# victorca25/traiNNer

Hardware: AMD Instinct MI355X
Metric: HR images/sec (G+D step), ESRGAN x4 128->512 (higher is better)
Workload: dtype f32 (bf16x3)

## Files before the change

### include/trainner_hip.h

```cpp
#ifndef TRAINNER_HIP_H
#define TRAINNER_HIP_H

#include <stdint.h>

#ifdef __cplusplus
extern "C" {
#endif

#define TNR_OK 0
#define TNR_EINVAL (-1)
#define TNR_ELAUNCH (-2)

enum { TNR_ACT_NONE = 0, TNR_ACT_LRELU = 1, TNR_ACT_RELU = 2 };

enum {
    TNR_CONV_3x3 = 0,
    TNR_CONV_3x3_UP2 = 1,
    TNR_CONV_4x4_S2 = 2,
    TNR_DGRAD_4x4_S2 = 3,
    TNR_CONV_1x1 = 4,
    TNR_CONV_3x3_C4 = 5,
    TNR_CONV_7x7_C4 = 6
};

enum {
    TNR_PACK_FWD = 0,
    TNR_PACK_DGRAD_3x3 = 1,
    TNR_PACK_FWD_S2D = 2,
    TNR_PACK_DGRAD_S2 = 3,
    TNR_PACK_COL_FWD = 4,
    TNR_PACK_COL_DGRAD3 = 5,
    TNR_PACK_C4_FWD = 6,
    TNR_PACK_C4_DGRAD3 = 7
};

#define TNR_MMA_F32 0
#define TNR_MMA_BF16 1
#define TNR_MMA_BF16X3 2

typedef struct tnr_view {
    float *ptr;
    int32_t ctot;
    int32_t coff;
} tnr_view;

typedef struct tnr_conv_desc {
    tnr_view x;
    int32_t N, H, W;
    int32_t Cin;
    const float *wp;
    int32_t KinP, KoutP;
    tnr_view y;
    int32_t Ho, Wo, Cout;
    int32_t mode;
    const float *bias;
    int32_t act;
// ... 74 lines not shown
int tnr_conv_sweep_pack_batch(const tnr_sweep_pack_item *items_dev, int32_t n, int32_t max_units, void *stream);
int tnr_conv_sweep(const tnr_conv_desc *stages, int32_t n, const void *image, uint32_t *ws, int64_t ws_bytes, uint32_t epoch,
                   void *stream);
int64_t tnr_conv_thin_pack_floats(int32_t reduce_channels);
int tnr_conv_thin_pack(const float *w_oihw, float *wp, int32_t Cout, int32_t Cin, int32_t dgrad, void *stream);
int tnr_conv_thin(tnr_view x, int32_t N, int32_t H, int32_t W, int32_t Cin, const float *wp, tnr_view y, int32_t Cout,
                  const float *bias, float alpha, void *stream);
int64_t tnr_conv_thin7_pack_floats(int32_t reduce_channels);
int tnr_conv_thin7_pack(const float *w_oihw, float *wp, int32_t Cout, int32_t Cin, int32_t dgrad, void *stream);
int tnr_conv_thin7(tnr_view x, int32_t N, int32_t H, int32_t W, int32_t Cin, const float *wp, tnr_view y, int32_t Ho, int32_t Wo,
                   int32_t Cout, int32_t pad, int32_t reflect, const float *bias, float alpha, void *stream);
int64_t tnr_wgrad_workspace_bytes(const tnr_wgrad_desc *d);
int64_t tnr_wgrad_thin_workspace_bytes(int32_t N, int32_t H, int32_t Cbig);
int tnr_wgrad_thin(tnr_view big, tnr_view small, int32_t N, int32_t H, int32_t W, int32_t Cbig, int32_t Csmall, int32_t flip,
                   float *dw, float *db, float alpha, float beta, float *ws, int64_t ws_bytes, void *stream);
int64_t tnr_wgrad_thin7_workspace_bytes(int32_t N, int32_t Hbig_grid, int32_t Cbig);
int tnr_wgrad_thin7(tnr_view big, int32_t N, int32_t H, int32_t W, int32_t rpad, tnr_view small, int32_t Hs, int32_t Ws, int32_t off,
                    int32_t Cbig, int32_t Csmall, int32_t flip, float *dw, float *db, float alpha, float beta, float *ws, int64_t ws_bytes,
                    void *stream);
int tnr_conv_wgrad(const tnr_wgrad_desc *d, void *stream);
#define TNR_WGRAD_GROUP_MAX 12
int tnr_conv_wgrad_group(const tnr_wgrad_desc *descs, int32_t n, void *stream);
int tnr_wgrad_tile_class(const tnr_wgrad_desc *d, int32_t group_jobs, int32_t x3_occ, int32_t out[12]);

int tnr_gconv_fwd(tnr_view x, int32_t N, int32_t H, int32_t W, int32_t Cin, const float *w, const float *bias, tnr_view y, int32_t Ho,
                  int32_t Wo, int32_t Cout, int32_t k, int32_t stride, int32_t pad, int32_t reflect, int32_t act, float slope, void *stream);
int tnr_gconv_dgrad(tnr_view g, int32_t N, int32_t H, int32_t W, int32_t Cin, const float *w, tnr_view gx, int32_t Ho, int32_t Wo,
                    int32_t Cout, int32_t k, int32_t stride, int32_t pad, int32_t reflect, void *stream);
int64_t tnr_gconv_wgrad_workspace_bytes(int32_t Cout, int32_t Cin, int32_t k);
int tnr_gconv_wgrad(tnr_view x, int32_t N, int32_t H, int32_t W, int32_t Cin, tnr_view g, int32_t Ho, int32_t Wo, int32_t Cout, int32_t k,
                    int32_t stride, int32_t pad, int32_t reflect, float *dw, float *db, float alpha, float beta, double *ws,
                    int64_t ws_bytes, void *stream);
int tnr_bias_grad(tnr_view g, int64_t pixels, int32_t C, float *db, float alpha, float beta, double *ws, int64_t ws_bytes, void *stream);
int tnr_pad2d(tnr_view x, tnr_view y, int32_t N, int32_t H, int32_t W, int32_t C, int32_t pad, int32_t mode, void *stream);
int tnr_unpad2d(tnr_view xp, tnr_view y, int32_t N, int32_t H, int32_t W, int32_t C, int32_t pad, int32_t mode, void *stream);
int tnr_window2d(tnr_view src, int32_t Hs, int32_t Ws, tnr_view dst, int32_t N, int32_t Hd, int32_t Wd, int32_t C, int32_t oy,
                 int32_t ox, int32_t acc, void *stream);
int tnr_tanh_fwd(const float *x, float *y, int64_t n, void *stream);
int tnr_tanh_bwd(const float *g, const float *y, float *gx, int64_t n, void *stream);
int tnr_gan_loss(const float *pred, int64_t n, int32_t type, float target, float *out, float *grad, void *stream);
int tnr_dp_unique_id(void *id128);
int tnr_dp_init(const void *id128, int32_t rank, int32_t world, void **comm);
int tnr_dp_allreduce_bucket(void *comm, float *buf, int64_t count, int32_t average, void *stream);
int tnr_dp_broadcast(void *comm, float *buf, int64_t count, int32_t root, void *stream);
int tnr_dp_comm_count(void *comm, int32_t *nranks);
int tnr_dp_finalize(void *comm);
// ... 178 lines not shown
```

### trainner_amd/csrc/conv_sweep.hip

```cpp
#include <stddef.h>
#include <string.h>
#include <type_traits>
#include <utility>
#include "conv_body.h"
#include "conv_epilogue.h"
#include "conv_handoff.h"

namespace {

constexpr int SW_TH = 8, SW_TW = 32, SW_HT = SW_TH + 2, SW_WT = SW_TW + 2;
constexpr int SW_ROW = TNR_X3_ROW;
constexpr int SW_A_ROWS = SW_HT * SW_WT;
constexpr int SW_A_ALLOC_ROWS = 384;
constexpr int SW_A_FLOATS = SW_A_ALLOC_ROWS * SW_ROW;
constexpr int SW_UNIT_FLOATS = 32 * SW_ROW;
constexpr int SW_SLOT_UNITS = 9;
constexpr int SW_SLOT_FLOATS = SW_SLOT_UNITS * SW_UNIT_FLOATS;
constexpr int SW_RING = 3;
constexpr size_t SW_LDS_BYTES = (size_t)(2 * SW_A_FLOATS + SW_RING * SW_SLOT_FLOATS) * sizeof(float);
constexpr int SW_NPASS = 9, SW_NSTAGE = 5, SW_NTILE = 6;
constexpr int SW_A_IT = (SW_A_ROWS * 4 + 511) / 512;
constexpr int SW_B_PIECES = (SW_SLOT_UNITS * 3 + 7) / 8;
static_assert(SW_LDS_BYTES <= 160 * 1024, "one sweep workgroup per CU");

// ... 1455 lines not shown
    const int form = sweep_form();
    if (n == SW4_NSTAGE) {
        TNR_REQUIRE(form == 5, "conv_sweep: four stages run in the direct four-wave form only");
        hipLaunchKernelGGL((conv_sweep4_kernel<true, false, SwPlan4>), dim3((unsigned)grid), dim3(256), S4D_LDS_BYTES, (hipStream_t)stream, c);
        return tnr_check_launch("conv_sweep");
    }
    if (stages[0].mma == TNR_MMA_BF16) {
        TNR_REQUIRE(form == 5, "conv_sweep: bf16 operands (use_amp) run in the direct four-wave form only");
        hipLaunchKernelGGL((conv_sweep4_kernel<true, true>), dim3((unsigned)grid), dim3(256), S4D_LDS_BYTES, (hipStream_t)stream, c);
        return tnr_check_launch("conv_sweep");
    }
    if (form == 8) hipLaunchKernelGGL(conv_sweep_kernel, dim3((unsigned)grid), dim3(512), SW_LDS_BYTES, (hipStream_t)stream, c);
    else if (form == 4) hipLaunchKernelGGL(conv_sweep4_kernel<false>, dim3((unsigned)grid), dim3(256), SW_LDS_BYTES, (hipStream_t)stream, c);
    else hipLaunchKernelGGL(conv_sweep4_kernel<true>, dim3((unsigned)grid), dim3(256), S4D_LDS_BYTES, (hipStream_t)stream, c);
    return tnr_check_launch("conv_sweep");
}

extern "C" int64_t tnr_conv_wq_bytes(const tnr_conv_desc *d) {
    if (d != nullptr && s2_ok(d)) return (int64_t)(d->Cout / 64) * (d->Cin / 16) * 4 * S2_NU * SW_UNIT_FLOATS * (int64_t)sizeof(float);
    if (d == nullptr || !d4_ok(d)) return 0;
    return (int64_t)(d->Cout / 64) * (d->Cin / 16) * 18 * SW_UNIT_FLOATS * (int64_t)sizeof(float);
}

extern "C" int tnr_conv_wq_pack(const tnr_conv_desc *d, void *image, int64_t image_bytes, void *stream) {
    if (d != nullptr && image != nullptr && d->wp != nullptr && s2_ok(d)) {
        S2PackK a;
        a.wp = d->wp; a.KinP = d->KinP; a.KoutP = d->KoutP; a.nck = d->Cin / 16; a.ncb = d->Cout / 64;
        a.dgrad = d->mode == TNR_DGRAD_4x4_S2;
        a.units = a.ncb * 4 * a.nck * S2_NU;
        TNR_REQUIRE((int64_t)a.units * SW_UNIT_FLOATS * (int64_t)sizeof(float) <= image_bytes, "conv_wq_pack: image buffer too small");
        a.out = static_cast<float *>(image);
        hipLaunchKernelGGL(s2_pack_kernel, dim3((unsigned)tnr_cdiv(a.units * 64, 256)), dim3(256), 0, (hipStream_t)stream, a);
        return tnr_check_launch("conv_wq_pack (four-tap form)");
    }
    TNR_REQUIRE(d != nullptr && image != nullptr && d->wp != nullptr && d4_ok(d), "conv_wq_pack: the launch cannot use a pre-split weight stream");
    D4PackK a;
    a.wp = d->wp; a.KinP = d->KinP; a.KoutP = d->KoutP; a.nck = d->Cin / 16; a.ncb = d->Cout / 64;
    a.units = a.ncb * a.nck * 18;
    a.shuffle = d->shuffle;
    TNR_REQUIRE((int64_t)a.units * SW_UNIT_FLOATS * (int64_t)sizeof(float) <= image_bytes, "conv_wq_pack: image buffer too small");
    a.out = static_cast<float *>(image);
    hipLaunchKernelGGL(d4_pack_kernel, dim3((unsigned)tnr_cdiv(a.units * 64, 256)), dim3(256), 0, (hipStream_t)stream, a);
    return tnr_check_launch("conv_wq_pack");
}

int tnr_launch_conv_s2_d4(const tnr_conv_desc *d, void *stream) {
// ... 43 lines not shown
```

### trainner_amd/csrc/pack_api.hip

```cpp
#include <stdarg.h>
#include <string.h>
#include "common.h"

static thread_local char g_err[512] = "";

void tnr_set_error(const char *fmt, ...) {
    va_list ap;
    va_start(ap, fmt);
    vsnprintf(g_err, sizeof(g_err), fmt, ap);
    va_end(ap);
}

int tnr_check_launch(const char *what) {
    hipError_t e = hipGetLastError();
    if (e != hipSuccess) {
        tnr_set_error("%s: %s", what, hipGetErrorString(e));
        return TNR_ELAUNCH;
    }
    return TNR_OK;
}

extern "C" const char *tnr_last_error(void) { return g_err; }

static unsigned *g_fault_word = nullptr;
// ... 27 lines not shown
            TNR_REQUIRE(kh == 4 && kw == 4, "pack dgrad s2: kernel must be 4x4");
            ko = tnr_round_up(Cin, 32); ki = tnr_round_up(Cout, TNR_CK);
            n = (int64_t)16 * ko * ki;
            break;
        case TNR_PACK_COL_FWD:
            ko = tnr_round_up(Cout, 32); ki = tnr_round_up(kh * kw * Cin, TNR_CK);
            n = (int64_t)ko * ki;
            break;
        case TNR_PACK_COL_DGRAD3:
            TNR_REQUIRE(kh == kw && kh >= 1, "pack col dgrad: kernel must be square");
            ko = tnr_round_up(Cin, 32); ki = tnr_round_up(kh * kw * Cout, TNR_CK);
            n = (int64_t)ko * ki;
            break;
        case TNR_PACK_C4_FWD:
            TNR_REQUIRE(kh == kw && (kh == 3 || kh == 7) && Cin <= 4, "pack c4: 3x3 or 7x7 kernel with Cin <= 4");
            ko = tnr_round_up(Cout, 32); ki = tnr_round_up(4 * kh * kw, TNR_CK);
            n = (int64_t)ko * ki;
            break;
        case TNR_PACK_C4_DGRAD3:
            TNR_REQUIRE(kh == kw && (kh == 3 || kh == 7) && Cout <= 4, "pack c4 dgrad: 3x3 or 7x7 kernel with Cout <= 4");
            ko = tnr_round_up(Cin, 32); ki = tnr_round_up(4 * kh * kw, TNR_CK);
            n = (int64_t)ko * ki;
            break;
        default:
            tnr_set_error("pack: bad kind %d", kind);
            return TNR_EINVAL;
    }
    if (KoutP) *KoutP = ko;
    if (KinP) *KinP = ki;
    if (n_out) *n_out = n;
    return TNR_OK;
}

namespace {
__global__ void pack_weights_kernel(const tnr_pack_item *items) {
    const tnr_pack_item it = items[blockIdx.y];
    const int Cout = it.Cout, Cin = it.Cin, kh = it.kh, kw = it.kw, ko = it.KoutP, ki = it.KinP;
    for (int64_t e = (int64_t)blockIdx.x * blockDim.x + threadIdx.x; e < it.n_out; e += (int64_t)gridDim.x * blockDim.x) {
        float v = 0.f;
        if (it.kind == TNR_PACK_FWD) {
            const int ci = (int)(e % ki);
            int64_t q = e / ki;
            const int co = (int)(q % ko);
            const int t = (int)(q / ko);
            if (co < Cout && ci < Cin) v = it.w[((size_t)co * Cin + ci) * kh * kw + t];
        } else if (it.kind == TNR_PACK_DGRAD_3x3) {
            const int co = (int)(e % ki);
            int64_t q = e / ki;
            const int ci = (int)(q % ko);
            const int t = (int)(q / ko);
            const int ky = 2 - t / 3, kx = 2 - t % 3;
            if (co < Cout && ci < Cin) v = it.w[(((size_t)co * Cin + ci) * 3 + ky) * 3 + kx];
        } else if (it.kind == TNR_PACK_FWD_S2D) {
            const int vch = (int)(e % (4 * ki));
            int64_t q = e / (4 * ki);
            const int co = (int)(q % ko);
            const int t = (int)(q / ko);
            const int pp = vch / ki, ci = vch - pp * ki;
            const int ky = 2 * (t >> 1) + (pp >> 1), kx = 2 * (t & 1) + (pp & 1);
            if (co < Cout && ci < Cin) v = it.w[(((size_t)co * Cin + ci) * 4 + ky) * 4 + kx];
        } else if (it.kind == TNR_PACK_COL_FWD) {
            const int v_ = (int)(e % ki);
            const int co = (int)(e / ki);
            const int t = v_ / Cin, ci = v_ - t * Cin;
            if (co < Cout && t < kh * kw) v = it.w[((size_t)co * Cin + ci) * kh * kw + t];
        } else if (it.kind == TNR_PACK_COL_DGRAD3) {
            const int v_ = (int)(e % ki);
            const int ci = (int)(e / ki);
            const int t = v_ / Cout, co = v_ - t * Cout;
            if (ci < Cin && t < kh * kw) v = it.w[(((size_t)co * Cin + ci) * kh + (kh - 1 - t / kw)) * kw + (kw - 1 - t % kw)];
        } else if (it.kind == TNR_PACK_C4_FWD) {
            const int v_ = (int)(e % ki);
            const int co = (int)(e / ki);
            const int t = v_ >> 2, ci = v_ & 3;
            if (co < Cout && t < kh * kw && ci < Cin) v = it.w[((size_t)co * Cin + ci) * kh * kw + t];
        } else if (it.kind == TNR_PACK_C4_DGRAD3) {
            const int v_ = (int)(e % ki);
            const int ci = (int)(e / ki);
            const int t = v_ >> 2, co = v_ & 3;
            if (ci < Cin && t < kh * kw && co < Cout) v = it.w[(((size_t)co * Cin + ci) * kh + (kh - 1 - t / kw)) * kw + (kw - 1 - t % kw)];
        } else {
            const int co = (int)(e % ki);
            int64_t q = e / ki;
            const int ci = (int)(q % ko);
            q /= ko;
            const int t = (int)(q & 3);
            const int par = (int)(q >> 2);
            const int py = par >> 1, px = par & 1;
            const int ky = ((py + 1) & 1) + 2 * (t >> 1), kx = ((px + 1) & 1) + 2 * (t & 1);
            if (co < Cout && ci < Cin) v = it.w[(((size_t)co * Cin + ci) * 4 + ky) * 4 + kx];
        }
        it.wp[e] = v;
    }
}
}

namespace {
__global__ void pack_dense_kernel(const tnr_dense_pack_item *items) {
    const tnr_dense_pack_item it = items[blockIdx.y];
    const int nf = it.nf, gc = it.gc, t = it.t, ko = it.KoutP, ki = it.KinP;
    const int ntarget = (t == 4) ? nf : gc;
    const int tlo = (t == 4) ? 0 : nf + (3 - t) * gc;
    const int K = nf + t * gc;
// ... 28 lines not shown
    if (KoutP) *KoutP = ko;
    if (KinP) *KinP = ki;
    if (n_out) *n_out = (int64_t)9 * ko * ki;
    return TNR_OK;
}

extern "C" int tnr_pack_dense_dgrad(const tnr_dense_pack_item *items_dev, int32_t n, int64_t max_out, void *stream) {
    TNR_REQUIRE(items_dev != nullptr && n > 0 && max_out > 0, "pack_dense: bad arguments");
    int64_t bx = tnr_cdiv64(max_out, 256 * 4);
    if (bx > 1024) bx = 1024;
    if (bx < 1) bx = 1;
    hipLaunchKernelGGL(pack_dense_kernel, dim3((unsigned)bx, (unsigned)n), dim3(256), 0, (hipStream_t)stream, items_dev);
    return tnr_check_launch("pack_dense_dgrad");
}

extern "C" int tnr_pack_weights(const tnr_pack_item *items_dev, int32_t n, int64_t max_out, void *stream) {
    TNR_REQUIRE(items_dev != nullptr && n > 0 && max_out > 0, "pack: bad arguments");
    int64_t bx = tnr_cdiv64(max_out, 256 * 4);
    if (bx > 1024) bx = 1024;
    if (bx < 1) bx = 1;
    hipLaunchKernelGGL(pack_weights_kernel, dim3((unsigned)bx, (unsigned)n), dim3(256), 0, (hipStream_t)stream, items_dev);
    return tnr_check_launch("pack_weights");
}
```

### trainner_amd/engine.py

```python
import torch

from . import hip, ops
from .flat import FlatParams


class ConvOp:

    def __init__(self, mod, packer, need_dgrad=True, ups=False):
        self.mod, self.packer = mod, packer
        k, s = mod.kernel_size, mod.stride
        if k == 3 and s == 1:
            self.mode_f = ops.CONV_3x3_UP2 if ups else ops.CONV_3x3
            self.mode_d = ops.CONV_3x3
            pf, pd = ops.PACK_FWD, ops.PACK_DGRAD_3x3
        elif k == 4 and s == 2 and not ups:
            self.mode_f, self.mode_d = ops.CONV_4x4_S2, ops.DGRAD_4x4_S2
            pf, pd = ops.PACK_FWD_S2D, ops.PACK_DGRAD_S2
        else:
            raise NotImplementedError("conv k=%d s=%d is not on the SR hot path" % (k, s))
        self.i_f = packer.add(mod.weight, pf)
        self.i_d = packer.add(mod.weight, pd) if need_dgrad else None
        deep = mod.in_channels * k * k >= 2048 and not ups
        i_fc = packer.add(mod.weight, ops.PACK_COL_FWD) if deep else None
        i_dc = packer.add(mod.weight, ops.PACK_COL_DGRAD3) if (deep and need_dgrad and k == 3) else None
        img = k == 3 and s == 1 and not ups
        self.thin = img
        i_f4 = packer.add(mod.weight, ops.PACK_C4_FWD) if (img and mod.in_channels <= 4) else None
        i_d4 = packer.add(mod.weight, ops.PACK_C4_DGRAD3) if (img and need_dgrad and mod.out_channels <= 4) else None
        cin, cout = mod.in_channels, mod.out_channels
        self.dirs = {False: (self.mode_f, ops.ConvLayer(k, s, cin, cout, False, ups, direct=self.i_f, c4=i_f4, col=i_fc)),
                     True: (self.mode_d, ops.ConvLayer(k, s, cin, cout, True, ups, direct=self.i_d, c4=i_d4, col=i_dc))}

    def _run(self, dgrad, x, y, epi):
        mode, layer = self.dirs[dgrad]
        wp = self.packer.get(layer.direct)
        form = ops.conv_plan(x, wp, y, mode, epi, layer=layer)[0]
        if form == "thin":
            ops.conv_thin(x, self.mod.weight, y, bias=None if dgrad else self.mod.bias, alpha=epi.get("alpha", 1.0), dgrad=dgrad)
        elif form == "c4":
            ops.conv(x if x.C == 4 else ops.View(x.buf), self.packer.get(layer.c4), y, mode=ops.CONV_3x3_C4, **epi)
        elif form == "im2col":
            ops.conv_small(x, self.packer.get(layer.col), y, layer.k, layer.stride, **epi)
        else:
            ops.conv(x, wp, y, mode=mode, **epi)

    def fwd(self, x, y, **epi):
        epi["bias"] = self.mod.bias
        self._run(False, x, y, epi)

    def fwd_shuffle2(self, x, y, **epi):
        return ops.conv_shuffle2(x, self.packer.get(self.i_f), y, layer=self.dirs[False][1], bias=self.mod.bias, **epi)

    def dgrad(self, g, gx, **epi):
        self._run(True, g, gx, epi)

    def fwd_stage(self, x, y, fresh_from=None, **epi):
        return dict(x=x, wp=self.packer.get(self.i_f), y=y, mode=self.mode_f, bias=self.mod.bias, fresh_from=fresh_from, **epi)

    def wgrad_item(self, x, g, alpha=1.0, cin_begin=0, with_bias=True, reflect=False):
        w = self.mod.weight
        db = self.mod.bias.grad if (with_bias and self.mod.bias is not None and cin_begin == 0) else None
        return dict(x=x, g=g, dw=w.grad, db=db, cin_begin=cin_begin, alpha=alpha, beta=1.0, reflect=reflect)

    def wgrad(self, x, g, alpha=1.0, cin_begin=0, with_bias=True, reflect=False):
        if reflect:
            ops.wgrad_group([self.wgrad_item(x, g, alpha, cin_begin, with_bias, reflect=True)], mode=self.mode_f)
            return
        if self.thin and ops.IMAGE_C4 and cin_begin == 0 and x.N == g.N and (x.H, x.W) == (g.H, g.W):
            m = self.mod
            db = m.bias.grad if (with_bias and m.bias is not None) else None
            if m.in_channels <= 3 and x.ctot == 4 and x.coff == 0 and g.C in (16, 32, 64):
                ops.wgrad_thin(g, ops.View(x.buf), m.weight.grad, db, flip=False, alpha=alpha)
                return
            if m.out_channels <= 3 and g.ctot == 4 and g.coff == 0 and x.C in (16, 32, 64):
                ops.wgrad_thin(x, ops.View(g.buf), m.weight.grad, db, flip=True, alpha=alpha)
                return
        ops.wgrad_group([self.wgrad_item(x, g, alpha, cin_begin, with_bias)], mode=self.mode_f)


class _NetFn(torch.autograd.Function):

    @staticmethod
    def forward(ctx, net, x, *params):
        need_param_grad = any(ctx.needs_input_grad[2:])
        need_graph = ctx.needs_input_grad[1] or need_param_grad
        memo = net._memo_lookup(x) if (net.memoize and net.training) else None
        if memo is not None and memo[1] is not None:
            out, saved = memo
            net.replay_forward_side_effects(saved)
# ... 92 lines not shown
```

### trainner_amd/hip.py

```python
import ctypes as C
import os

import torch

from . import build as _build

c_f = C.c_float
c_i = C.c_int32
c_l = C.c_int64
c_p = C.c_void_p

ACT_NONE, ACT_LRELU, ACT_RELU = 0, 1, 2
MMA_F32, MMA_BF16, MMA_BF16X3 = 0, 1, 2
CONV_3x3, CONV_3x3_UP2, CONV_4x4_S2, DGRAD_4x4_S2, CONV_1x1, CONV_3x3_C4, CONV_7x7_C4 = 0, 1, 2, 3, 4, 5, 6
PACK_FWD, PACK_DGRAD_3x3, PACK_FWD_S2D, PACK_DGRAD_S2, PACK_COL_FWD, PACK_COL_DGRAD3 = 0, 1, 2, 3, 4, 5
PACK_C4_FWD, PACK_C4_DGRAD3 = 6, 7
PACK_DENSE_DGRAD = 16


class CView(C.Structure):
    _fields_ = [("ptr", c_p), ("ctot", c_i), ("coff", c_i)]


class ConvDesc(C.Structure):
    _fields_ = [
        ("x", CView), ("N", c_i), ("H", c_i), ("W", c_i), ("Cin", c_i),
        ("wp", c_p), ("KinP", c_i), ("KoutP", c_i),
        ("y", CView), ("Ho", c_i), ("Wo", c_i), ("Cout", c_i),
        ("mode", c_i), ("bias", c_p), ("act", c_i), ("slope", c_f), ("alpha", c_f),
        ("r1", CView), ("r1_ch", c_i), ("beta1", c_f),
        ("r2", CView), ("alpha2", c_f),
        ("m", CView), ("m_lo", c_i), ("m_hi", c_i), ("m_slope", c_f),
        ("ws", c_p), ("ws_bytes", c_l), ("mma", c_i), ("pad_mode", c_i),
        ("noise_sigma", c_f), ("noise_pos", c_i), ("noise_key0", C.c_uint32), ("noise_key1", C.c_uint32), ("noise_pix0", C.c_uint32),
        ("wq", c_p), ("wq_bytes", c_l), ("wq_form", c_i), ("shuffle", c_i),
    ]


class WgradDesc(C.Structure):
# ... 38 lines not shown
    "tnr_gauss_mult": (c_i, [CView, CView, c_l, c_i, c_f, C.c_uint32, C.c_uint32, C.c_uint32, c_p]),
    "tnr_im2col": (c_i, [CView, c_i, c_i, c_i, c_i, c_i, c_i, c_i, c_i, c_i, c_p, c_p]),
    "tnr_conv_chain_workspace_bytes": (c_l, [C.POINTER(ConvDesc)]),
    "tnr_conv_chain": (c_i, [C.POINTER(ConvDesc), C.POINTER(C.c_int32), c_i, c_p, c_l, C.c_uint32, c_p]),
    "tnr_conv_sweep_image_bytes": (c_l, [C.POINTER(ConvDesc), c_i]),
    "tnr_conv_sweep_pack_item": (c_i, [C.POINTER(ConvDesc), c_i, c_p, c_l, C.POINTER(SweepPackItem)]),
    "tnr_conv_sweep_pack_batch": (c_i, [c_p, c_i, c_i, c_p]),
    "tnr_conv_sweep_pack": (c_i, [C.POINTER(ConvDesc), c_i, c_p, c_l, c_p]),
    "tnr_conv_sweep": (c_i, [C.POINTER(ConvDesc), c_i, c_p, c_p, c_l, C.c_uint32, c_p]),
    "tnr_conv_thin_pack_floats": (c_l, [c_i]),
    "tnr_conv_thin_pack": (c_i, [c_p, c_p, c_i, c_i, c_i, c_p]),
    "tnr_conv_thin": (c_i, [CView, c_i, c_i, c_i, c_i, c_p, CView, c_i, c_p, c_f, c_p]),
    "tnr_wgrad_workspace_bytes": (c_l, [C.POINTER(WgradDesc)]),
    "tnr_conv_thin7_pack_floats": (c_l, [c_i]),
    "tnr_conv_thin7_pack": (c_i, [c_p, c_p, c_i, c_i, c_i, c_p]),
    "tnr_conv_thin7": (c_i, [CView, c_i, c_i, c_i, c_i, c_p, CView, c_i, c_i, c_i, c_i, c_i, c_p, c_f, c_p]),
    "tnr_wgrad_thin7_workspace_bytes": (c_l, [c_i, c_i, c_i]),
    "tnr_wgrad_thin7": (c_i, [CView, c_i, c_i, c_i, c_i, CView, c_i, c_i, c_i, c_i, c_i, c_i, c_p, c_p, c_f, c_f, c_p, c_l, c_p]),
    "tnr_wgrad_thin_workspace_bytes": (c_l, [c_i, c_i, c_i]),
    "tnr_wgrad_thin": (c_i, [CView, CView, c_i, c_i, c_i, c_i, c_i, c_i, c_p, c_p, c_f, c_f, c_p, c_l, c_p]),
    "tnr_conv_wgrad": (c_i, [C.POINTER(WgradDesc), c_p]),
    "tnr_conv_wgrad_group": (c_i, [C.POINTER(WgradDesc), c_i, c_p]),
    "tnr_wgrad_tile_class": (c_i, [C.POINTER(WgradDesc), c_i, c_i, C.POINTER(c_i * 12)]),
    "tnr_nchw_to_nhwc": (c_i, [c_p, c_i, c_i, c_i, c_i, CView, c_i, c_p, c_p, c_p]),
    "tnr_nhwc_to_nchw": (c_i, [CView, c_i, c_i, c_i, c_i, c_p, c_p, c_i, c_p]),
    "tnr_upsample2x_bwd": (c_i, [CView, CView, c_i, c_i, c_i, c_i, CView, c_f, c_p]),
    "tnr_depth_to_space": (c_i, [CView, CView, c_i, c_i, c_i, c_i, c_p]),
    "tnr_space_to_depth_bwd": (c_i, [CView, CView, c_i, c_i, c_i, c_i, CView, c_f, c_p]),
    "tnr_maxpool2_fwd": (c_i, [CView, CView, c_i, c_i, c_i, c_i, c_p]),
    "tnr_maxpool2_bwd": (c_i, [CView, CView, CView, c_i, c_i, c_i, c_i, c_p]),
    "tnr_gconv_fwd": (c_i, [CView, c_i, c_i, c_i, c_i, c_p, c_p, CView, c_i, c_i, c_i, c_i, c_i, c_i, c_i, c_i, c_f, c_p]),
    "tnr_gconv_dgrad": (c_i, [CView, c_i, c_i, c_i, c_i, c_p, CView, c_i, c_i, c_i, c_i, c_i, c_i, c_i, c_p]),
    "tnr_gconv_wgrad_workspace_bytes": (c_l, [c_i, c_i, c_i]),
    "tnr_gconv_wgrad": (c_i, [CView, c_i, c_i, c_i, c_i, CView, c_i, c_i, c_i, c_i, c_i, c_i, c_i, c_p, c_p, c_f, c_f, c_p, c_l, c_p]),
    "tnr_bias_grad": (c_i, [CView, c_l, c_i, c_p, c_f, c_f, c_p, c_l, c_p]),
    "tnr_pad2d": (c_i, [CView, CView, c_i, c_i, c_i, c_i, c_i, c_i, c_p]),
    "tnr_unpad2d": (c_i, [CView, CView, c_i, c_i, c_i, c_i, c_i, c_i, c_p]),
    "tnr_window2d": (c_i, [CView, c_i, c_i, CView, c_i, c_i, c_i, c_i, c_i, c_i, c_i, c_p]),
    "tnr_tanh_fwd": (c_i, [c_p, c_p, c_l, c_p]),
    "tnr_tanh_bwd": (c_i, [c_p, c_p, c_p, c_l, c_p]),
    "tnr_gan_loss": (c_i, [c_p, c_l, c_i, c_f, c_p, c_p, c_p]),
    "tnr_dp_unique_id": (c_i, [c_p]),
    "tnr_dp_init": (c_i, [c_p, c_i, c_i, C.POINTER(c_p)]),
    "tnr_dp_allreduce_bucket": (c_i, [c_p, c_p, c_l, c_i, c_p]),
    "tnr_dp_broadcast": (c_i, [c_p, c_p, c_l, c_i, c_p]),
    "tnr_dp_comm_count": (c_i, [c_p, C.POINTER(c_i)]),
# ... 159 lines not shown
```

### trainner_amd/models/modules/architectures/RRDBNet_arch.py

```python
import math

import torch
import torch.nn as nn

from .... import ops
from ....engine import ConvOp, HipNet
from ....ops import View, new_act
from . import block as B


class ResidualDenseBlock_5C(nn.Module):
    def __init__(self, nf=64, gc=32, act_type="leakyrelu"):
        super().__init__()
        self.conv1 = B.conv_block(nf, gc, 3, act_type=act_type)
        self.conv2 = B.conv_block(nf + gc, gc, 3, act_type=act_type)
        self.conv3 = B.conv_block(nf + 2 * gc, gc, 3, act_type=act_type)
        self.conv4 = B.conv_block(nf + 3 * gc, gc, 3, act_type=act_type)
        self.conv5 = B.conv_block(nf + 4 * gc, nf, 3, act_type=None)


class RRDB(nn.Module):
    def __init__(self, nf, gc=32, act_type="leakyrelu"):
        super().__init__()
        self.RDB1 = ResidualDenseBlock_5C(nf, gc, act_type)
# ... 201 lines not shown
        sched = getattr(self, "_bucket_schedule", None) if W else None

        def done(op):
            if sched is not None:
                sched.mark_done(op.mod.weight)

        if W:
            o["hr1"].wgrad(h0, View(g4, 0, self.out_nc))
            done(o["hr1"])
        gcur = View(new_act(N, cur.H, cur.W, nf, dev))
        last_stage = sv["stages"][-1] if sv["stages"] else None
        o["hr0"].dgrad(gh0, gcur, **(dict(mask=cur, m_slope=sl) if (last_stage and self.upsample_mode == "upconv") else {}))
        if W:
            o["hr0"].wgrad(cur, gh0)
            done(o["hr0"])
        for si in range(len(sv["stages"]) - 1, -1, -1):
            src, dst, t = sv["stages"][si]
            u = o["up"][si]
            prev_is_act = si > 0 and self.upsample_mode == "upconv"
            if self.upsample_mode == "upconv":
                if W:
                    u.wgrad(src, gcur)
                    done(u)
                gup = View(new_act(N, dst.H, dst.W, nf, dev))
                u.dgrad(gcur, gup)
                gsrc = View(new_act(N, src.H, src.W, nf, dev))
                ops.upsample2x_bwd(gup, gsrc, mask=(src if prev_is_act else None), mslope=sl)
            else:
                gt = View(new_act(N, src.H, src.W, 4 * nf, dev))
                ops.space_to_depth_bwd(gcur, gt, mask=dst, mslope=sl)
                if W:
                    u.wgrad(src, gt)
                    done(u)
                gsrc = View(new_act(N, src.H, src.W, nf, dev))
                u.dgrad(gt, gsrc)
            gcur = gsrc
        gy0 = gcur
        nrdb = 3 * self.nb
        cb = nf + 4 * gc
        G = [new_act(N, h, w, cb, dev) for _ in range(4 if nrdb else 1)]
        if W:
            o["lr"].wgrad(View(sv["trunk"]), gy0)
            done(o["lr"])
        nz = sv.get("noise")
        P = [View(new_act(N, h, w, nf, dev)) for _ in range(2)] if (nz and nrdb) else None
        pc = 0
        o["lr"].dgrad(gy0, P[0] if P else View(G[0], 0, nf))
        if P:
            ops.gauss_mult(View(G[0], 0, nf), P[0], nz[nrdb - 1])
        pin = 0
# ... 33 lines not shown
```

### trainner_amd/ops.py

```python
import collections
import ctypes as C

import os

import torch

from . import hip
from .hip import (ACT_LRELU, ACT_NONE, ACT_RELU, CONV_1x1, CONV_3x3, CONV_3x3_C4, CONV_3x3_UP2, CONV_4x4_S2, CONV_7x7_C4, DGRAD_4x4_S2,
                  PACK_C4_DGRAD3, PACK_C4_FWD, PACK_COL_DGRAD3, PACK_COL_FWD, PACK_DENSE_DGRAD, PACK_DGRAD_3x3, PACK_DGRAD_S2, PACK_FWD, PACK_FWD_S2D, CView,
                  ConvDesc,
                  DensePackItem, PackItem, WgradDesc)


def round_up(a, b):
    return (a + b - 1) // b * b


class View:
    __slots__ = ("buf", "coff", "C")

    def __init__(self, buf, coff=0, C=None):
        assert buf.dim() == 4 and buf.dtype == torch.float32 and buf.is_contiguous()
        self.buf, self.coff = buf, coff
        self.C = buf.shape[3] - coff if C is None else C
        assert 0 <= coff and coff + self.C <= buf.shape[3]

    N = property(lambda s: s.buf.shape[0])
    H = property(lambda s: s.buf.shape[1])
    W = property(lambda s: s.buf.shape[2])
    ctot = property(lambda s: s.buf.shape[3])
    pixels = property(lambda s: s.buf.shape[0] * s.buf.shape[1] * s.buf.shape[2])

# ... 230 lines not shown


def noise_key(seed, call, block):
    M = 0xFFFFFFFFFFFFFFFF

    def mix(z):
        z = (z + 0x9E3779B97F4A7C15) & M
        z = ((z ^ (z >> 30)) * 0xBF58476D1CE4E5B9) & M
        z = ((z ^ (z >> 27)) * 0x94D049BB133111EB) & M
        return z ^ (z >> 31)

    return mix(mix(mix(seed & M) ^ (call & M)) ^ (block & M))


def gauss_mult(dst, src, noise):
    hip.check(hip.load().tnr_gauss_mult(dst.c(), cv(src), dst.pixels, dst.C, noise.sigma, noise.key0, noise.key1, noise.pix0,
                                        hip.stream()), "gauss_mult")


IMAGE_C4 = os.environ.get("TNR_IMAGE_C4", "1") != "0"
SMALL_GEMM = os.environ.get("TNR_SMALL_GEMM", "1") != "0"
S2_D4 = os.environ.get("TNR_S2_D4", "1") != "0"
X3_D4 = os.environ.get("TNR_X3_D4", "1") != "0"
_wq_oneoff = {}
_sweep_images = {}
_ONEOFF_IMAGES = {"_wq_images": _wq_oneoff, "_sweep_images": _sweep_images}


def _stream_image(owner, attr, key, need, dev, pack):
    if owner is None:
        cache, gen, key = _ONEOFF_IMAGES[attr], None, (key, hip.stream())
    else:
        cache, gen = owner.__dict__.setdefault(attr, {}), owner.gen
    ent = cache.get(key)
    if owner is None and ent is not None:
        cache[key] = cache.pop(key)
    fresh = ent is None or ent[0].numel() * 4 < need
    if fresh:
        ent = cache[key] = [torch.empty(need // 4, dtype=torch.float32, device=dev), None]
        if owner is None:
            while len(cache) > 64:
                cache.pop(next(iter(cache)))
    if gen is None or ent[1] != gen:
        pack(ent[0].data_ptr(), need)
        ent[1] = gen
    return ent, fresh
# ... 61 lines not shown
    if mode in (CONV_3x3_C4, CONV_7x7_C4):
        return "c4", why
    if mode == CONV_3x3:
        no = ((wino is False and "forbidden")
              or (wino is None and not WINO and "switch")
              or (wino is None and (x.C < WINO_MIN_CIN or y.pixels < WINO_MIN_PIXELS) and "shape")
              or (mma != hip.MMA_BF16X3 and "arithmetic")
              or (y.C % 64 and "shape")
              or (not wino_ok and "declined"))
        if not no:
            return "wino", why or ("forced" if wino else None)
        why = why or no
    if mode in (CONV_3x3, CONV_4x4_S2, DGRAD_4x4_S2):
        no = ((not (X3_D4 and (S2_D4 or mode == CONV_3x3)) and "switch")
              or (mma not in _STREAM_MMA and "arithmetic")
              or (y.C % 64 and "shape")
              or (not stream_ok and "declined"))
        if not no:
            return "stream", why
        why = why or no
    return "tile", why


def _conv_launch(x, wp, y, mode, wino, shuffle, epi, layer=None):
    d, said = None, {}
    while True:
        form, why = conv_plan(x, wp, y, mode, epi, shuffle, layer, wino, **said)
        if shuffle and form != "stream":
            return None
        if d is None:
            lib, d = hip.load(), ConvDesc()
            _conv_desc(d, x, wp, y, mode, **epi)
            if shuffle:
                d.Ho, d.Wo, d.Cout, d.shuffle, d.m_hi = x.H, x.W, 4 * y.C, shuffle, 0
        if why == "splitk":
            need = lib.tnr_conv_workspace_bytes(C.byref(d))
            if need > 0:
                ws = WS.get("splitk@%x" % hip.stream(), need, x.buf.device)
                d.ws, d.ws_bytes = ws.data_ptr(), ws.numel() * 8
                break
            said["splitk"] = False
        elif form == "wino":
            img = _wino_image(lib, d, wp, x.buf.device)
            if img is not None:
                d.wq, d.wq_bytes, d.wq_form = img.data_ptr(), img.numel() * 4, 1
                break
            assert wino is not True, "this launch cannot run in the Winograd form"
            said["wino_ok"] = False
        elif form == "stream":
            img = _wq_image(lib, d, wp, x.buf.device, tag="shuffle2" if shuffle else None)
            if img is not None:
                d.wq, d.wq_bytes = img.data_ptr(), img.numel() * 4
                break
            said["stream_ok"] = False
        else:
            break
    t0 = PROFILE.begin() if PROFILE is not None else None
    hip.check(lib.tnr_conv_forward(C.byref(d), hip.stream()), "conv_forward")
    if PROFILE is not None:
        fam, taps = _CONV_FAMILY[mode]
        PROFILE.end("conv_wino_3x3" if form == "wino" else fam, 2.0 * d.N * d.Ho * d.Wo * taps * min(x.C, wp.KinP) * d.Cout, t0, (x.C, d.Cout, d.Ho, wp.kind))
    return form


def conv_shuffle2(x, wp, y, layer=None, **epi):
    return _conv_launch(x, wp, y, CONV_3x3, None, 2, epi, layer) is not None


def conv(x, wp, y, mode=CONV_3x3, wino=None, **epi):
    _conv_launch(x, wp, y, mode, wino, 0, epi)


CHAIN_MAX = 6
CONV_CHAIN = os.environ.get("TNR_CONV_CHAIN", "1") != "0"
CONV_SWEEP = os.environ.get("TNR_CONV_SWEEP", "1") != "0"
CHAIN_X3 = os.environ.get("TNR_CHAIN_X3", "1") == "1"
AMP_SWEEP = os.environ.get("TNR_AMP_SWEEP", "1") != "0"
SWEEP_DISPENSED = os.environ.get("TNR_SWEEP_WAVES", "4") != "8"
CHAIN_WITH_COLLECTIVES = os.environ.get("TNR_CHAIN_WITH_COLLECTIVES", "0") == "1"
SWEEP_AUTO = os.environ.get("TNR_SWEEP_AUTO", "1") != "0"
SWEEP_AUTO_STATE = {"choice": None, "sweep_us": None, "layers_us": None}
DENSE_SPLIT = os.environ.get("TNR_DENSE_SPLIT", "1") != "0"
_SWEEP_FORM_DMA = os.environ.get("TNR_SWEEP_FORM", "")[:2] == "dm"
COLLECTIVES_IN_FLIGHT = False
COUNTERS = {"one_launch_next_to_collectives": 0, "per_layer_next_to_collectives": 0}
_cu_counts = {}


def _cus(dev):
    if dev not in _cu_counts:
        _cu_counts[dev] = torch.cuda.get_device_properties(dev).multi_processor_count
    return _cu_counts[dev]

# ... 311 lines not shown
WGRAD_X3 = os.environ.get("TNR_WGRAD_X3", "1") == "1"


def _wgrad_desc(d, x, g, dw, db, mode, cin_begin, alpha, beta, reflect=False, pair=None):
    d.x = x.c()
    d.N, d.H, d.W, d.Cin = x.N, x.H, x.W, x.C
    d.g = g.c()
    d.Ho, d.Wo, d.Cout = g.H, g.W, g.C
    d.mode = mode
    d.dw, d.cin_total, d.cin_begin = dw.data_ptr(), dw.shape[1], cin_begin
    d.db = hip.ptr(db)
    d.alpha, d.beta = alpha, beta
    d.mma = hip.MMA_F32 if (MMA == hip.MMA_BF16X3 and not WGRAD_X3) else MMA
    d.pad_mode = 1 if reflect else 0
    if pair is not None:
        dw2, db2, split = pair
        d.dw2, d.cin_total2, d.cout_split, d.db2 = dw2.data_ptr(), dw2.shape[1], split, hip.ptr(db2)


def wgrad(x, g, dw, db=None, mode=CONV_3x3, cin_begin=0, alpha=1.0, beta=1.0, reflect=False):
    wgrad_group([dict(x=x, g=g, dw=dw, db=db, cin_begin=cin_begin, alpha=alpha, beta=beta, reflect=reflect)], mode=mode)


def wgrad_group(items, mode=CONV_3x3):
    lib = hip.load()
    n = len(items)
    assert 1 <= n <= WGRAD_GROUP_MAX
    descs = (WgradDesc * n)()
    for d, it in zip(descs, items):
        _wgrad_desc(d, it["x"], it["g"], it["dw"], it.get("db"), mode, it.get("cin_begin", 0),
                    it.get("alpha", 1.0), it.get("beta", 1.0), it.get("reflect", False), it.get("pair"))
    dev = items[0]["x"].buf.device
    for i, d in enumerate(descs):
        need = lib.tnr_wgrad_workspace_bytes(C.byref(d))
        ws = WS.get("wgrad%d" % i, need, dev)
        d.ws, d.ws_bytes = ws.data_ptr(), ws.numel() * 8
    if PROFILE is None:
        hip.check(lib.tnr_conv_wgrad_group(descs, n, hip.stream()), "conv_wgrad_group")
        return
    t0 = PROFILE.begin()
    hip.check(lib.tnr_conv_wgrad_group(descs, n, hip.stream()), "conv_wgrad_group")
    taps = 16 if mode == CONV_4x4_S2 else 9
    x0, g0 = items[0]["x"], items[0]["g"]
    flops = sum(2.0 * it["g"].pixels * taps * it["x"].C * it["g"].C for it in items)
    PROFILE.end("wgrad_tile", flops, t0, (sum(it["x"].C for it in items) if n > 1 else x0.C, g0.C, g0.H, mode + 100 * (n - 1)))


def wgrad_tile_class(desc, group_jobs=0, x3_occ=-1):
    out = (C.c_int32 * 12)()
    hip.check(hip.load().tnr_wgrad_tile_class(C.byref(desc), group_jobs, x3_occ, C.byref(out)), "wgrad_tile_class")
    return dict(zip(("mode", "a_t", "b_t", "thg", "bf", "wps", "db", "ks", "splits", "tiles_per_split", "lds", "row"), out))


def wgrad_thin(big, small4, dw, db, flip, alpha=1.0, beta=1.0):
    lib = hip.load()
    cs = dw.shape[0] if flip else dw.shape[1]
    need = lib.tnr_wgrad_thin_workspace_bytes(big.N, big.H, big.C)
    ws = WS.get("wgrad_thin@%x" % hip.stream(), need, big.buf.device)
    t0 = PROFILE.begin() if PROFILE is not None else None
    hip.check(lib.tnr_wgrad_thin(big.c(), small4.c(), big.N, big.H, big.W, big.C, cs, int(flip), dw.data_ptr(), hip.ptr(db),
                                 alpha, beta, ws.data_ptr(), ws.numel() * 8, hip.stream()), "wgrad_thin")
    if PROFILE is not None:
        PROFILE.end("wgrad_thin", 2.0 * big.pixels * 9 * big.C * cs, t0, (big.C, cs, big.H, int(flip)))


def nchw_to_nhwc(src, dst, Cpad=None, scale=None, shift=None):
    N, Cc, H, W = src.shape
    assert src.is_contiguous() and src.dtype == torch.float32
# ... 486 lines not shown
```

Before: 73.08.

## Fold nearest-upsample into 3x3 conv as stride-2 transposed 4x4 conv

Measured after the change: 73.76 (median of 6 runs). No clear change (+0.9%).

```diff
diff --git a/include/trainner_hip.h b/include/trainner_hip.h
--- a/include/trainner_hip.h
+++ b/include/trainner_hip.h
@@ -31,7 +31,9 @@
     TNR_PACK_COL_FWD = 4,
     TNR_PACK_COL_DGRAD3 = 5,
     TNR_PACK_C4_FWD = 6,
-    TNR_PACK_C4_DGRAD3 = 7
+    TNR_PACK_C4_DGRAD3 = 7,
+    TNR_PACK_UP2_FWD = 8,
+    TNR_PACK_UP2_DGRAD = 9
 };
 
 #define TNR_MMA_F32 0
@@ -152,6 +154,8 @@
 #define TNR_WGRAD_GROUP_MAX 12
 int tnr_conv_wgrad_group(const tnr_wgrad_desc *descs, int32_t n, void *stream);
 int tnr_wgrad_tile_class(const tnr_wgrad_desc *d, int32_t group_jobs, int32_t x3_occ, int32_t out[12]);
+int tnr_up2_fold_ok(int32_t Cin, int32_t Cout, int32_t H, int32_t W, int32_t mma, int32_t dgrad);
+int tnr_up2_unfold_wgrad(const float *dk, float *dw, int32_t Cout, int32_t Cin, float alpha, float beta, void *stream);
 
 int tnr_gconv_fwd(tnr_view x, int32_t N, int32_t H, int32_t W, int32_t Cin, const float *w, const float *bias, tnr_view y, int32_t Ho,
                   int32_t Wo, int32_t Cout, int32_t k, int32_t stride, int32_t pad, int32_t reflect, int32_t act, float slope, void *stream);
diff --git a/trainner_amd/csrc/conv_sweep.hip b/trainner_amd/csrc/conv_sweep.hip
--- a/trainner_amd/csrc/conv_sweep.hip
+++ b/trainner_amd/csrc/conv_sweep.hip
@@ -1501,6 +1501,25 @@
     return (int64_t)(d->Cout / 64) * (d->Cin / 16) * 18 * SW_UNIT_FLOATS * (int64_t)sizeof(float);
 }
 
+extern "C" int tnr_up2_fold_ok(int32_t Cin, int32_t Cout, int32_t H, int32_t W, int32_t mma, int32_t dgrad) {
+    if (mma != TNR_MMA_BF16X3) return 0;
+    if (Cin <= 0 || Cout <= 0 || H <= 0 || W <= 0 || H > (1 << 14) || W > (1 << 14)) return 0;
+    tnr_conv_desc d;
+    memset(&d, 0, sizeof(d));
+    d.N = 1;
+    d.mma = mma;
+    if (dgrad) {
+        d.mode = TNR_CONV_4x4_S2;
+        d.H = 2 * H; d.W = 2 * W; d.Cin = d.KinP = d.x.ctot = Cout;
+        d.Ho = H; d.Wo = W; d.Cout = d.KoutP = d.y.ctot = Cin;
+    } else {
+        d.mode = TNR_DGRAD_4x4_S2;
+        d.H = H; d.W = W; d.Cin = d.KinP = d.x.ctot = Cin;
+        d.Ho = 2 * H; d.Wo = 2 * W; d.Cout = d.KoutP = d.y.ctot = Cout;
+    }
+    return s2_ok(&d) ? 1 : 0;
+}
+
 extern "C" int tnr_conv_wq_pack(const tnr_conv_desc *d, void *image, int64_t image_bytes, void *stream) {
     if (d != nullptr && image != nullptr && d->wp != nullptr && s2_ok(d)) {
         S2PackK a;
diff --git a/trainner_amd/csrc/pack_api.hip b/trainner_amd/csrc/pack_api.hip
--- a/trainner_amd/csrc/pack_api.hip
+++ b/trainner_amd/csrc/pack_api.hip
@@ -73,6 +73,16 @@
             ko = tnr_round_up(Cin, 32); ki = tnr_round_up(4 * kh * kw, TNR_CK);
             n = (int64_t)ko * ki;
             break;
+        case TNR_PACK_UP2_FWD:
+            TNR_REQUIRE(kh == 3 && kw == 3, "pack up2 fwd: kernel must be 3x3");
+            ko = tnr_round_up(Cout, 32); ki = tnr_round_up(Cin, TNR_CK);
+            n = (int64_t)16 * ko * ki;
+            break;
+        case TNR_PACK_UP2_DGRAD:
+            TNR_REQUIRE(kh == 3 && kw == 3, "pack up2 dgrad: kernel must be 3x3");
+            ko = tnr_round_up(Cin, 32); ki = tnr_round_up(Cout, TNR_CK);
+            n = (int64_t)4 * ko * 4 * ki;
+            break;
         default:
             tnr_set_error("pack: bad kind %d", kind);
             return TNR_EINVAL;
@@ -84,6 +94,13 @@
 }
 
 namespace {
+__device__ inline float up2_fold(const float *w9, int a, int b) {
+    double s = 0.0;
+    for (int ky = (a < 2 ? 2 - a : 0); ky <= (a > 0 ? 3 - a : 2); ++ky)
+        for (int kx = (b < 2 ? 2 - b : 0); kx <= (b > 0 ? 3 - b : 2); ++kx) s += (double)w9[ky * 3 + kx];
+    return (float)s;
+}
+
 __global__ void pack_weights_kernel(const tnr_pack_item *items) {
     const tnr_pack_item it = items[blockIdx.y];
     const int Cout = it.Cout, Cin = it.Cin, kh = it.kh, kw = it.kw, ko = it.KoutP, ki = it.KinP;
@@ -130,6 +147,24 @@
             const int ci = (int)(e / ki);
             const int t = v_ >> 2, co = v_ & 3;
             if (ci < Cin && t < kh * kw && co < Cout) v = it.w[(((size_t)co * Cin + ci) * kh + (kh - 1 - t / kw)) * kw + (kw - 1 - t % kw)];
+        } else if (it.kind == TNR_PACK_UP2_DGRAD) {
+            const int vch = (int)(e % (4 * ki));
+            int64_t q = e / (4 * ki);
+            const int ci = (int)(q % ko);
+            const int t = (int)(q / ko);
+            const int pp = vch / ki, co = vch - pp * ki;
+            const int a = 2 * (t >> 1) + (pp >> 1), b = 2 * (t & 1) + (pp & 1);
+            if (co < Cout && ci < Cin) v = up2_fold(it.w + ((size_t)co * Cin + ci) * 9, a, b);
+        } else if (it.kind == TNR_PACK_UP2_FWD) {
+            const int ci = (int)(e % ki);
+            int64_t q = e / ki;
+            const int co = (int)(q % ko);
+            q /= ko;
+            const int t = (int)(q & 3);
+            const int par = (int)(q >> 2);
+            const int py = par >> 1, px = par & 1;
+            const int a = ((py + 1) & 1) + 2 * (t >> 1), b = ((px + 1) & 1) + 2 * (t & 1);
+            if (co < Cout && ci < Cin) v = up2_fold(it.w + ((size_t)co * Cin + ci) * 9, a, b);
         } else {
             const int co = (int)(e % ki);
             int64_t q = e / ki;
@@ -204,3 +239,25 @@
     hipLaunchKernelGGL(pack_weights_kernel, dim3((unsigned)bx, (unsigned)n), dim3(256), 0, (hipStream_t)stream, items_dev);
     return tnr_check_launch("pack_weights");
 }
+
+namespace {
+__global__ void up2_unfold_wgrad_kernel(const float *dk, float *dw, int Cout, int Cin, float alpha, float beta) {
+    const int e = blockIdx.x * blockDim.x + threadIdx.x;
+    if (e >= Cout * Cin * 9) return;
+    const int kx = e % 3, ky = (e / 3) % 3, ci = (e / 9) % Cin, co = e / (9 * Cin);
+    const float *k = dk + ((size_t)ci * Cout + co) * 16 + (2 - ky) * 4 + (2 - kx);
+    float s = k[0];
+    s += k[1];
+    s += k[4];
+    s += k[5];
+    const float prev = (beta != 0.f) ? beta * dw[e] : 0.f;
+    dw[e] = prev + alpha * s;
+}
+}
+
+extern "C" int tnr_up2_unfold_wgrad(const float *dk, float *dw, int32_t Cout, int32_t Cin, float alpha, float beta, void *stream) {
+    TNR_REQUIRE(dk != nullptr && dw != nullptr && Cout > 0 && Cin > 0 && (int64_t)Cout * Cin * 16 < (1LL << 31), "up2_unfold_wgrad: bad arguments");
+    hipLaunchKernelGGL(up2_unfold_wgrad_kernel, dim3((unsigned)tnr_cdiv(Cout * Cin * 9, 256)), dim3(256), 0, (hipStream_t)stream, dk, dw, Cout, Cin,
+                       alpha, beta);
+    return tnr_check_launch("up2_unfold_wgrad");
+}
diff --git a/trainner_amd/engine.py b/trainner_amd/engine.py
--- a/trainner_amd/engine.py
+++ b/trainner_amd/engine.py
@@ -27,6 +27,8 @@
         self.thin = img
         i_f4 = packer.add(mod.weight, ops.PACK_C4_FWD) if (img and mod.in_channels <= 4) else None
         i_d4 = packer.add(mod.weight, ops.PACK_C4_DGRAD3) if (img and need_dgrad and mod.out_channels <= 4) else None
+        self.i_uf = packer.add(mod.weight, ops.PACK_UP2_FWD) if ups else None
+        self.i_ud = packer.add(mod.weight, ops.PACK_UP2_DGRAD) if (ups and need_dgrad) else None
         cin, cout = mod.in_channels, mod.out_channels
         self.dirs = {False: (self.mode_f, ops.ConvLayer(k, s, cin, cout, False, ups, direct=self.i_f, c4=i_f4, col=i_fc)),
                      True: (self.mode_d, ops.ConvLayer(k, s, cin, cout, True, ups, direct=self.i_d, c4=i_d4, col=i_dc))}
@@ -44,8 +46,14 @@
         else:
             ops.conv(x, wp, y, mode=mode, **epi)
 
+    def _folds(self, lo, direction):
+        return self.i_uf is not None and ops.up2_fold_plan(lo, self.mod.in_channels, self.mod.out_channels, direction)[0] == "fold"
+
     def fwd(self, x, y, **epi):
         epi["bias"] = self.mod.bias
+        if self._folds(x, 1):
+            ops.conv(x, self.packer.get(self.i_uf), y, mode=ops.DGRAD_4x4_S2, family="conv_up2_fold", **epi)
+            return
         self._run(False, x, y, epi)
 
     def fwd_shuffle2(self, x, y, **epi):
@@ -53,6 +61,12 @@
 
     def dgrad(self, g, gx, **epi):
         self._run(True, g, gx, epi)
+
+    def dgrad_lowres(self, g, gx, **epi):
+        if self.i_ud is None or not self._folds(gx, 2):
+            return False
+        ops.conv(g, self.packer.get(self.i_ud), gx, mode=ops.CONV_4x4_S2, family="conv_up2_fold", **epi)
+        return True
 
     def fwd_stage(self, x, y, fresh_from=None, **epi):
         return dict(x=x, wp=self.packer.get(self.i_f), y=y, mode=self.mode_f, bias=self.mod.bias, fresh_from=fresh_from, **epi)
@@ -65,6 +79,10 @@
     def wgrad(self, x, g, alpha=1.0, cin_begin=0, with_bias=True, reflect=False):
         if reflect:
             ops.wgrad_group([self.wgrad_item(x, g, alpha, cin_begin, with_bias, reflect=True)], mode=self.mode_f)
+            return
+        if cin_begin == 0 and self._folds(x, 4):
+            it = self.wgrad_item(x, g, alpha, 0, with_bias)
+            ops.wgrad_up2_fold(x, g, it["dw"], it["db"], alpha=alpha, beta=1.0)
             return
         if self.thin and ops.IMAGE_C4 and cin_begin == 0 and x.N == g.N and (x.H, x.W) == (g.H, g.W):
             m = self.mod
diff --git a/trainner_amd/hip.py b/trainner_amd/hip.py
--- a/trainner_amd/hip.py
+++ b/trainner_amd/hip.py
@@ -15,6 +15,7 @@
 CONV_3x3, CONV_3x3_UP2, CONV_4x4_S2, DGRAD_4x4_S2, CONV_1x1, CONV_3x3_C4, CONV_7x7_C4 = 0, 1, 2, 3, 4, 5, 6
 PACK_FWD, PACK_DGRAD_3x3, PACK_FWD_S2D, PACK_DGRAD_S2, PACK_COL_FWD, PACK_COL_DGRAD3 = 0, 1, 2, 3, 4, 5
 PACK_C4_FWD, PACK_C4_DGRAD3 = 6, 7
+PACK_UP2_FWD, PACK_UP2_DGRAD = 8, 9
 PACK_DENSE_DGRAD = 16
 
 
@@ -99,6 +100,8 @@
     "tnr_conv_wgrad": (c_i, [C.POINTER(WgradDesc), c_p]),
     "tnr_conv_wgrad_group": (c_i, [C.POINTER(WgradDesc), c_i, c_p]),
     "tnr_wgrad_tile_class": (c_i, [C.POINTER(WgradDesc), c_i, c_i, C.POINTER(c_i * 12)]),
+    "tnr_up2_fold_ok": (c_i, [c_i, c_i, c_i, c_i, c_i, c_i]),
+    "tnr_up2_unfold_wgrad": (c_i, [c_p, c_p, c_i, c_i, c_f, c_f, c_p]),
     "tnr_nchw_to_nhwc": (c_i, [c_p, c_i, c_i, c_i, c_i, CView, c_i, c_p, c_p, c_p]),
     "tnr_nhwc_to_nchw": (c_i, [CView, c_i, c_i, c_i, c_i, c_p, c_p, c_i, c_p]),
     "tnr_upsample2x_bwd": (c_i, [CView, CView, c_i, c_i, c_i, c_i, CView, c_f, c_p]),
diff --git a/trainner_amd/models/modules/architectures/RRDBNet_arch.py b/trainner_amd/models/modules/architectures/RRDBNet_arch.py
--- a/trainner_amd/models/modules/architectures/RRDBNet_arch.py
+++ b/trainner_amd/models/modules/architectures/RRDBNet_arch.py
@@ -247,10 +247,11 @@
                 if W:
                     u.wgrad(src, gcur)
                     done(u)
-                gup = View(new_act(N, dst.H, dst.W, nf, dev))
-                u.dgrad(gcur, gup)
                 gsrc = View(new_act(N, src.H, src.W, nf, dev))
-                ops.upsample2x_bwd(gup, gsrc, mask=(src if prev_is_act else None), mslope=sl)
+                if not u.dgrad_lowres(gcur, gsrc, **(dict(mask=src, m_slope=sl) if prev_is_act else {})):
+                    gup = View(new_act(N, dst.H, dst.W, nf, dev))
+                    u.dgrad(gcur, gup)
+                    ops.upsample2x_bwd(gup, gsrc, mask=(src if prev_is_act else None), mslope=sl)
             else:
                 gt = View(new_act(N, src.H, src.W, 4 * nf, dev))
                 ops.space_to_depth_bwd(gcur, gt, mask=dst, mslope=sl)
diff --git a/trainner_amd/ops.py b/trainner_amd/ops.py
--- a/trainner_amd/ops.py
+++ b/trainner_amd/ops.py
@@ -7,7 +7,7 @@
 
 from . import hip
 from .hip import (ACT_LRELU, ACT_NONE, ACT_RELU, CONV_1x1, CONV_3x3, CONV_3x3_C4, CONV_3x3_UP2, CONV_4x4_S2, CONV_7x7_C4, DGRAD_4x4_S2,
-                  PACK_C4_DGRAD3, PACK_C4_FWD, PACK_COL_DGRAD3, PACK_COL_FWD, PACK_DENSE_DGRAD, PACK_DGRAD_3x3, PACK_DGRAD_S2, PACK_FWD, PACK_FWD_S2D, CView,
+                  PACK_C4_DGRAD3, PACK_C4_FWD, PACK_COL_DGRAD3, PACK_COL_FWD, PACK_DENSE_DGRAD, PACK_DGRAD_3x3, PACK_DGRAD_S2, PACK_FWD, PACK_FWD_S2D, PACK_UP2_DGRAD, PACK_UP2_FWD, CView,
                   ConvDesc,
                   DensePackItem, PackItem, WgradDesc)
 
@@ -284,6 +284,7 @@
 SMALL_GEMM = os.environ.get("TNR_SMALL_GEMM", "1") != "0"
 S2_D4 = os.environ.get("TNR_S2_D4", "1") != "0"
 X3_D4 = os.environ.get("TNR_X3_D4", "1") != "0"
+UP2_FOLD = int(os.environ.get("TNR_UP2_FOLD", "6"))
 _wq_oneoff = {}
 _sweep_images = {}
 _ONEOFF_IMAGES = {"_wq_images": _wq_oneoff, "_sweep_images": _sweep_images}
@@ -391,7 +392,17 @@
     return "tile", why
 
 
-def _conv_launch(x, wp, y, mode, wino, shuffle, epi, layer=None):
+def up2_fold_plan(lo, cin, cout, direction, mma=_LIVE, fold=_LIVE):
+    mma = MMA if mma is _LIVE else mma
+    fold = UP2_FOLD if fold is _LIVE else fold
+    prod, red = (cin, cout) if direction == 2 else (cout, cin)
+    no = ((not (fold & direction and X3_D4 and S2_D4 and lo.buf.is_cuda) and "switch")
+          or (mma != hip.MMA_BF16X3 and "arithmetic")
+          or ((prod % 64 or red % 16 or red < 32 or lo.H < 8 or lo.W < 32 or 4 * lo.H * lo.W * max(lo.ctot, cin, cout) >= 1 << 30) and "shape"))
+    return ("up2", no) if no else ("fold", None)
+
+
+def _conv_launch(x, wp, y, mode, wino, shuffle, epi, layer=None, family=None):
     d, said = None, {}
     while True:
         form, why = conv_plan(x, wp, y, mode, epi, shuffle, layer, wino, **said)
@@ -428,7 +439,7 @@
     hip.check(lib.tnr_conv_forward(C.byref(d), hip.stream()), "conv_forward")
     if PROFILE is not None:
         fam, taps = _CONV_FAMILY[mode]
-        PROFILE.end("conv_wino_3x3" if form == "wino" else fam, 2.0 * d.N * d.Ho * d.Wo * taps * min(x.C, wp.KinP) * d.Cout, t0, (x.C, d.Cout, d.Ho, wp.kind))
+        PROFILE.end("conv_wino_3x3" if form == "wino" else (family or fam), 2.0 * d.N * d.Ho * d.Wo * taps * min(x.C, wp.KinP) * d.Cout, t0, (x.C, d.Cout, d.Ho, wp.kind))
     return form
 
 
@@ -436,8 +447,8 @@
     return _conv_launch(x, wp, y, CONV_3x3, None, 2, epi, layer) is not None
 
 
-def conv(x, wp, y, mode=CONV_3x3, wino=None, **epi):
-    _conv_launch(x, wp, y, mode, wino, 0, epi)
+def conv(x, wp, y, mode=CONV_3x3, wino=None, family=None, **epi):
+    _conv_launch(x, wp, y, mode, wino, 0, epi, family=family)
 
 
 CHAIN_MAX = 6
@@ -795,7 +806,7 @@
     wgrad_group([dict(x=x, g=g, dw=dw, db=db, cin_begin=cin_begin, alpha=alpha, beta=beta, reflect=reflect)], mode=mode)
 
 
-def wgrad_group(items, mode=CONV_3x3):
+def wgrad_group(items, mode=CONV_3x3, family="wgrad_tile"):
     lib = hip.load()
     n = len(items)
     assert 1 <= n <= WGRAD_GROUP_MAX
@@ -816,7 +827,23 @@
     taps = 16 if mode == CONV_4x4_S2 else 9
     x0, g0 = items[0]["x"], items[0]["g"]
     flops = sum(2.0 * it["g"].pixels * taps * it["x"].C * it["g"].C for it in items)
-    PROFILE.end("wgrad_tile", flops, t0, (sum(it["x"].C for it in items) if n > 1 else x0.C, g0.C, g0.H, mode + 100 * (n - 1)))
+    PROFILE.end(family, flops, t0, (sum(it["x"].C for it in items) if n > 1 else x0.C, g0.C, g0.H, mode + 100 * (n - 1)))
+
+
+def up2_unfold_wgrad(dk, dw, alpha=1.0, beta=1.0):
+    Cout, Cin = dw.shape[:2]
+    assert tuple(dk.shape) == (Cin, Cout, 4, 4) and tuple(dw.shape[2:]) == (3, 3) and dk.is_contiguous() and dw.is_contiguous()
+    hip.check(hip.load().tnr_up2_unfold_wgrad(dk.data_ptr(), dw.data_ptr(), Cout, Cin, alpha, beta, hip.stream()), "up2_unfold_wgrad")
+
+
+def wgrad_up2_fold(x, g, dw, db=None, alpha=1.0, beta=1.0):
+    Cout, Cin = dw.shape[:2]
+    scr = WS.get("up2_fold_dk@%x" % hip.stream(), Cin * Cout * 16 * 4, x.buf.device)
+    dk = scr.view(torch.float32)[:Cin * Cout * 16].view(Cin, Cout, 4, 4)
+    wgrad_group([dict(x=g, g=x, dw=dk, db=None, alpha=1.0, beta=0.0)], mode=CONV_4x4_S2, family="wgrad_up2_fold")
+    up2_unfold_wgrad(dk, dw, alpha, beta)
+    if db is not None:
+        bias_grad(g, db, alpha, beta)
 
 
 def wgrad_tile_class(desc, group_jobs=0, x3_occ=-1):
```
